# mnesbit/ImageExperiments

Measured on AMD Instinct MI355X. Metric: encode Mpixels/s at quality=3.5, higher is better.
Workload: dtype f64; 1 GPU; 4928x3264 synthetic RGB, 8 distinct frames in turn (mt19937 seed 12345+f), quality 3.5, K=32 atoms/tile-channel, 8x8 tiles; container_bytes=6650795

## Files before the change

### imageexperiments_amd/csrc/mp_pursuit.hip

```cpp
#include <hip/hip_runtime.h>
#include <stdint.h>
#include <type_traits>

#include "mp_device.h"

namespace mpc {

namespace {

constexpr int N = 64;
constexpr int kGroups = 1;
constexpr int kWavesDouble = 12;
constexpr int kWavesFloat = 12;
constexpr int kWavesMax = 16;
constexpr int kTilesLds = kBaseFilterTiles + kBlockFilterTiles;
constexpr double W_R = 0.299, W_G = 0.587, W_B = 0.114;
constexpr double U_SCALE = 0.436 / (1.0 - 0.114);
constexpr double V_SCALE = 0.615 / (1.0 - 0.299);
#ifndef MPC_SLACK
#define MPC_SLACK 0x1p-13f
#endif
constexpr float kSlack = MPC_SLACK;
constexpr float kAbs = 0x1p-100f;
constexpr float kHuge = 1.0e30f;
// ... 40 lines not shown
    unsigned lo = (unsigned)__double2loint(x), hi = (unsigned)__double2hiint(x);
    const auto a = __builtin_amdgcn_permlane16_swap(lo, lo, false, false);
    const auto b = __builtin_amdgcn_permlane16_swap(hi, hi, false, false);
    const double m = __hiloint2double((int)b[0], (int)a[0]) + __hiloint2double((int)b[1], (int)a[1]);
    lo = (unsigned)__double2loint(m); hi = (unsigned)__double2hiint(m);
    const auto c = __builtin_amdgcn_permlane32_swap(lo, lo, false, false);
    const auto d = __builtin_amdgcn_permlane32_swap(hi, hi, false, false);
    return __hiloint2double((int)d[0], (int)c[0]) + __hiloint2double((int)d[1], (int)c[1]);
}
__device__ __forceinline__ double from_prev16(double x)
{
    const unsigned lo = (unsigned)__double2loint(x), hi = (unsigned)__double2hiint(x);
    const auto a = __builtin_amdgcn_permlane16_swap(lo, lo, false, false);
    const auto b = __builtin_amdgcn_permlane16_swap(hi, hi, false, false);
    return __hiloint2double((int)b[0], (int)a[0]);
}
__device__ __forceinline__ double from_next16(double x)
{
    const unsigned lo = (unsigned)__double2loint(x), hi = (unsigned)__double2hiint(x);
    const auto a = __builtin_amdgcn_permlane16_swap(lo, lo, false, false);
    const auto b = __builtin_amdgcn_permlane16_swap(hi, hi, false, false);
    return __hiloint2double((int)b[1], (int)a[1]);
}
__device__ __forceinline__ double from_prev32(double x)
{
    const unsigned lo = (unsigned)__double2loint(x), hi = (unsigned)__double2hiint(x);
    const auto a = __builtin_amdgcn_permlane32_swap(lo, lo, false, false);
    const auto b = __builtin_amdgcn_permlane32_swap(hi, hi, false, false);
    return __hiloint2double((int)b[0], (int)a[0]);
}
__device__ __forceinline__ double from_next32(double x)
{
    const unsigned lo = (unsigned)__double2loint(x), hi = (unsigned)__double2hiint(x);
    const auto a = __builtin_amdgcn_permlane32_swap(lo, lo, false, false);
    const auto b = __builtin_amdgcn_permlane32_swap(hi, hi, false, false);
    return __hiloint2double((int)b[1], (int)a[1]);
}

__device__ __forceinline__ float from_prev16(float x) { return __uint_as_float(__builtin_amdgcn_permlane16_swap(__float_as_uint(x), __float_as_uint(x), false, false)[0]); }
__device__ __forceinline__ float from_next16(float x) { return __uint_as_float(__builtin_amdgcn_permlane16_swap(__float_as_uint(x), __float_as_uint(x), false, false)[1]); }
__device__ __forceinline__ float from_prev32(float x) { return __uint_as_float(__builtin_amdgcn_permlane32_swap(__float_as_uint(x), __float_as_uint(x), false, false)[0]); }
__device__ __forceinline__ float from_next32(float x) { return __uint_as_float(__builtin_amdgcn_permlane32_swap(__float_as_uint(x), __float_as_uint(x), false, false)[1]); }

__device__ __forceinline__ int pos_of(int h) { return h ^ (h >> 1); }

template <class T>
__device__ __forceinline__ T chain_sum(const T (&term)[16], int h)
{
    T t = 0;
#pragma unroll
    for (int i = 0; i < 16; ++i) t += term[i];
    T u = from_prev16(t);
#pragma unroll
    for (int i = 0; i < 16; ++i) u += term[i];
    t = h == 1 ? u : t;
    u = from_prev32(t);
#pragma unroll
    for (int i = 0; i < 16; ++i) u += term[i];
    t = h == 3 ? u : t;
    u = from_next16(t);
#pragma unroll
    for (int i = 0; i < 16; ++i) u += term[i];
    t = h == 2 ? u : t;
    u = from_prev16(t);
    t = h == 3 ? u : t;
    u = from_next32(t);
    return h < 2 ? u : t;
}

struct TopKeys {
    float k1 = 0.0f, k2 = 0.0f;
    __device__ __forceinline__ void see(unsigned value_bits, unsigned keep_mask, unsigned code)
    {
        const unsigned key = (value_bits & keep_mask) | code;
        k2 = __builtin_amdgcn_fmed3f(k1, k2, __uint_as_float(key));
        const unsigned k1b = __float_as_uint(k1);
        k1 = __uint_as_float(k1b > key ? k1b : key);
    }
};
__device__ __forceinline__ unsigned in_vgpr(unsigned x)
{
    unsigned v;
    asm volatile("v_mov_b32 %0, %1" : "=v"(v) : "s"(x));
    return v;
}
__device__ __forceinline__ unsigned in_sgpr(unsigned x)
{
    unsigned v;
    asm volatile("s_mov_b32 %0, %1" : "=s"(v) : "s"(x));
    return v;
}
constexpr unsigned kKeepRow = 0x7FFFFF80u;
constexpr unsigned kKeepPair = 0x7FFFFE00u;

struct Survivors {
    int q0 = 0, q1 = 0, q2 = 0, q3 = 0, count = 0;
    bool overflow = false;
    __device__ __forceinline__ void push(int code)
    {
        if (count == 0) q0 = code; else if (count == 1) q1 = code; else if (count == 2) q2 = code; else if (count == 3) q3 = code;
        else overflow = true;
        if (count < 4) ++count;
    }
    __device__ __forceinline__ int at(int i) const { return i == 0 ? q0 : (i == 1 ? q1 : (i == 2 ? q2 : q3)); }
};

struct TileChannel {
    int prev_id = 0;
    int next_off = 0;
    int off0 = 0;
    int npairs = 0;
    int fresh = -1;
    unsigned pk0 = 0, pk1 = 0;
    unsigned swept = 0;
    bool has0 = false, live = false;
    double coeff = 0.0;
    int sel_g = 0;
    int step = 0;
    int t = 0;
    __device__ __forceinline__ unsigned packed(int p) const { return ((p < 2 ? pk0 : pk1) >> (16 * (p & 1))) & 0xFFFFu; }
};

__device__ __forceinline__ void load16(double (&x)[16], const double* p)
{
    const double2* q = reinterpret_cast<const double2*>(p);
#pragma unroll
    for (int i = 0; i < 8; ++i) {
        const double2 v = q[i];
        x[2 * i] = v.x;
        x[2 * i + 1] = v.y;
    }
}

__device__ __forceinline__ void load16(float (&x)[16], const float* p)
{
    const float4* q = reinterpret_cast<const float4*>(p);
#pragma unroll
    for (int i = 0; i < 4; ++i) {
        const float4 v = q[i];
        x[4 * i] = v.x;
        x[4 * i + 1] = v.y;
        x[4 * i + 2] = v.z;
        x[4 * i + 3] = v.w;
    }
}

__device__ __forceinline__ double abs_of(double x) { return __builtin_fabs(x); }
__device__ __forceinline__ float abs_of(float x) { return __builtin_fabsf(x); }

template <class T>
__device__ __forceinline__ void keep_better(T& v, int& i, int& sel, T ov, int oi, int osel)
{
    const T a = abs_of(ov), b = abs_of(v);
    if (oi >= 0 && (a > b || (a == b && i >= 0 && oi < i))) {
        v = ov; i = oi; sel = osel;
    }
}

__device__ __forceinline__ int lane_id_fresh()
{
    int l;
    asm volatile("v_mbcnt_lo_u32_b32 %0, -1, 0\n\tv_mbcnt_hi_u32_b32 %0, -1, %0" : "=v"(l));
    return l;
}
#define FRESH_LANE                                                                    \
    const int lane = lane_id_fresh();                                                 \
    const int slot = lane & 15, h = lane >> 4;                                        \
    const int pix0 = 16 * pos_of(h);                                                  \
    (void)slot; (void)h; (void)pix0;

#ifdef MPC_STAMPS
#define STAMP(i)                                              \
// ... 38 lines not shown
            s_tiles[i] = i < kBaseFilterTiles * 256 ? src_base[i] : src_blk0[i - kBaseFilterTiles * 256];
        for (int i = threadIdx.x; i < 512; i += 64 * kWaves) {
            s_rows[i] = i < a.num_base ? a.block_rows[i] : 0;
            s_rowoff[i] = i < a.num_base ? a.block_row_off[i] : 0;
        }
        for (int i = threadIdx.x; i < 3 * kMaxDeviceK; i += 64 * kWaves)
            s_quant[i / kMaxDeviceK][i % kMaxDeviceK] = (i % kMaxDeviceK) < a.K ? a.quant[(i / kMaxDeviceK) * a.K + i % kMaxDeviceK] : 1.0;
        if (threadIdx.x == 0) {
            s_home = ch_first;
            s_on[0] = s_on[1] = s_on[2] = 0;
            s_on[ch_first] = kWaves;
        }
    }
    __syncthreads();

    const int wave = __builtin_amdgcn_readfirstlane((int)(threadIdx.x >> 6));
    int ch = ch_first;
    const T* detail = nullptr;
    const uint16_t* block_tiles = nullptr;
    const float* gram = nullptr;
    unsigned* queue = nullptr;
    long long n_tc = 0;
    auto bind_channel = [&](int c) {
        c = __builtin_amdgcn_readfirstlane(c);
        ch = c;
        detail = reinterpret_cast<const T*>(kFast ? static_cast<const void*>(c == 0 ? a.detail32[0] : (c == 1 ? a.detail32[1] : a.detail32[2]))
                                                  : static_cast<const void*>(c == 0 ? a.detail[0] : (c == 1 ? a.detail[1] : a.detail[2])));
        block_tiles = c == 0 ? a.block_tiles[0] : (c == 1 ? a.block_tiles[1] : a.block_tiles[2]);
        gram = c == 0 ? a.gram[0] : (c == 1 ? a.gram[1] : a.gram[2]);
        queue = a.queue + c;
        n_tc = c == 0 ? a.n_tc[0] : (c == 1 ? a.n_tc[1] : a.n_tc[2]);
    };
    bind_channel(ch_first);
    const long long wave_global = (long long)blockIdx.x * kWaves + wave;
    float* const my_p = a.pair_p + wave_global * (kGroups * 16 * kMaxPairs * 64);
    unsigned* const my_meta = a.pair_meta + wave_global * (kGroups * 16 * kMaxPairs * 2);
    float* const my_e = a.pair_e + wave_global * (kGroups * 16 * kMaxPairs);
    unsigned* const my_touch = s_touch + 64 * wave;
    const int K = a.K;

    const unsigned keep_row_mask = in_vgpr(kKeepRow), keep_pair_mask = in_vgpr(kKeepPair);
    unsigned n_mfma = 0, n_steps = 0;
    int unit[kGroups];
    T r[kGroups][16];
    TileChannel tc[kGroups];
#pragma unroll
    for (int g = 0; g < kGroups; ++g) {
        unit[g] = -1;
#pragma unroll
        for (int i = 0; i < 16; ++i) r[g][i] = 0;
    }
    bool queue_empty = false;

    auto tile_mfma = [&](const uint4 (&av)[4], const bf16x8 (&hi)[2], const bf16x8 (&lo)[2]) {
        f32x4 acc = {0.0f, 0.0f, 0.0f, 0.0f};
#pragma unroll
        for (int kk = 0; kk < 2; ++kk) {
            bf16x8 ah, al;
            __builtin_memcpy(&ah, &av[2 * kk + 0], 16);
            __builtin_memcpy(&al, &av[2 * kk + 1], 16);
            acc = __builtin_amdgcn_mfma_f32_16x16x32_bf16(ah, hi[kk], acc, 0, 0, 0);
            acc = __builtin_amdgcn_mfma_f32_16x16x32_bf16(ah, lo[kk], acc, 0, 0, 0);
            acc = __builtin_amdgcn_mfma_f32_16x16x32_bf16(al, hi[kk], acc, 0, 0, 0);
        }
        return acc;
    };
    auto rec_of = [&](int t) { return a.vec_in ? (long long)t : (long long)t * 3 + ch; };
    auto lds_tile = [&](uint4 (&dst)[4], int t, int lane) {
#pragma unroll
        for (int q = 0; q < 4; ++q) dst[q] = s_tiles[t * 256 + q * 64 + lane];
    };
    auto far_tile = [&](uint4 (&dst)[4], int t, int lane) {
        const uint4* tiles = reinterpret_cast<const uint4*>(block_tiles) + lane;
#pragma unroll
        for (int q = 0; q < 4; ++q) dst[q] = tiles[t * 256 + q * 64];
    };

    TopKeys tp[kGroups];
    float lbmax[kGroups];
    bool oddp[kGroups];
    float rbound[kGroups];
#pragma unroll
    for (int g = 0; g < kGroups; ++g) { lbmax[g] = -3.0e38f; oddp[g] = false; rbound[g] = 0.0f; }
    auto pair_update = [&](auto gc, auto same_p, int p, bool upd, unsigned info, float4 (&pv)[4], const float4 (&gv)[4], float E) {
        constexpr int g = decltype(gc)::value;
        FRESH_LANE
        const long long pi = (long long)(g * 16 + slot) * kMaxPairs + p;
        const int rows = (int)((info >> 9) & 127u);
        if (upd) {
            const float c32 = (float)tc[g].coeff;
            float4* pp = reinterpret_cast<float4*>(my_p + pi * 64 + 4 * h);
#pragma unroll
            for (int t = 0; t < 4; ++t) {
                pv[t].x = fmaf(-c32, gv[t].x, pv[t].x);
                pv[t].y = fmaf(-c32, gv[t].y, pv[t].y);
                pv[t].z = fmaf(-c32, gv[t].z, pv[t].z);
                pv[t].w = fmaf(-c32, gv[t].w, pv[t].w);
                pp[4 * t] = pv[t];
            }
            E = (E + 0x1p-21f * (fabsf(c32) + rbound[g])) * 1.000001f;
            if (h == 0) my_e[pi] = E;
            oddp[g] = oddp[g] || !(fabsf(c32) < kHuge);
        }
        oddp[g] = oddp[g] || !(E < kHuge);
        const bool pad2 = h == 3 && rows < 63, pad3 = h == 3 && rows < 64;
        const unsigned keepp = keep_pair_mask;
        float biggest = 0.0f;
#pragma unroll
        for (int t = 0; t < 4; ++t) {
            const float vals[4] = {pv[t].x, pv[t].y, pv[t].z, pv[t].w};
#pragma unroll
            for (int v = 0; v < 4; ++v) {
                const float m = fabsf(vals[v]);
                float ub = m + E;
                if (t == 3 && v == 2) ub = pad2 ? 0.0f : ub;
                if (t == 3 && v == 3) ub = pad3 ? 0.0f : ub;
                const unsigned code = (unsigned)((p << 4) | (t << 2) | v);
                tp[g].see(__float_as_uint(ub), keepp, decltype(same_p)::value ? in_sgpr((unsigned)__builtin_amdgcn_readfirstlane((int)code)) : code);
                biggest = __builtin_amdgcn_fmed3f(biggest, m, __builtin_inff());
            }
        }
        lbmax[g] = __builtin_amdgcn_fmed3f(lbmax[g], biggest - E, __builtin_inff());
    };
    for (;;) {
        bool any_unit = false;
        for (;;) {
        static_for<kGroups>([&](auto gc) {
            constexpr int g = decltype(gc)::value;
            if (queue_empty) return;
            const unsigned free_slots = (unsigned)(__ballot(!tc[g].live) & 0xFFFFull);
            const int n_free = __popc(free_slots);
            if (!(n_free >= kRefillAt || (unit[g] < 0 && n_free > 0))) return;
            FRESH_LANE
            int first = 0;
            if (lane == 0) first = (int)atomicAdd(queue, (unsigned)n_free);
            first = __builtin_amdgcn_readfirstlane(first);
            if ((long long)first + n_free >= n_tc) queue_empty = true;
            const long long t = (long long)first + __popc(free_slots & ((1u << slot) - 1u));
            const bool take = !tc[g].live && t < n_tc;
            if (!__ballot(take)) return;
            unit[g] = 0;
            TileChannel s;
            s.live = true;
            s.t = (int)t;
            s.next_off = a.num_base;
            const long long ts = take ? t : 0;
            T fresh_r[16];
            if (a.vec_in) {
                double in[16];
                load16(in, a.vec_in + ts * N + pix0);
#pragma unroll
                for (int i = 0; i < 16; ++i) fresh_r[i] = (T)in[i];
            } else {
                const int tiles_per_frame = a.tiles_x * a.tile_rows;
                const int frame = (int)(ts / tiles_per_frame);
                const int tile = (int)(ts - (long long)frame * tiles_per_frame);
                const int tx = tile / a.tile_rows, ty = a.tile_row_begin + (tile - tx * a.tile_rows);
                if (a.out_tile_rows > 0) s.t = (frame * a.tiles_x + tx) * a.out_tile_rows + ty;
                const uint8_t* img = a.rgb + (long long)frame * a.frame_stride;
                unsigned char px[16][3];
                const bool whole = tx * 8 + 8 <= a.width && ty * 8 + 8 <= a.height;
                if (a.rgb_aligned8 && !__ballot(!whole)) {
#pragma unroll
                    for (int rr = 0; rr < 2; ++rr) {
                        const uint2* p = reinterpret_cast<const uint2*>(img + (long long)(ty * 8 + (pix0 >> 3) + rr) * a.row_stride + 24 * tx);
                        const uint2 v0 = p[0], v1 = p[1], v2 = p[2];
                        const unsigned w[6] = {v0.x, v0.y, v1.x, v1.y, v2.x, v2.y};
#pragma unroll
                        for (int b = 0; b < 24; ++b) px[8 * rr + b / 3][b % 3] = (unsigned char)((w[b >> 2] >> (8 * (b & 3))) & 0xFFu);
                    }
                } else {
#pragma unroll
                    for (int i = 0; i < 16; ++i) {
                        const int x = tx * 8 + (i & 7), y = ty * 8 + (pix0 >> 3) + (i >> 3);
                        const int xc = x < a.width ? x : a.width - 1, yc = y < a.height ? y : a.height - 1;
                        const uint8_t* p = img + (long long)yc * a.row_stride + 3 * xc;
                        px[i][0] = p[0]; px[i][1] = p[1]; px[i][2] = p[2];
                    }
                }
#pragma unroll
                for (int i = 0; i < 16; ++i) {
                    const int x = tx * 8 + (i & 7), y = ty * 8 + (pix0 >> 3) + (i >> 3);
                    const double red = (double)px[i][0], green = (double)px[i][1], blue = (double)px[i][2];
                    const double Y = (W_R * red + W_G * green + W_B * blue);
                    const double v = ch == 0 ? Y : (ch == 1 ? (U_SCALE * (blue - Y)) : (V_SCALE * (red - Y)));
                    fresh_r[i] = (T)((x < a.width && y < a.height) ? v : 0.0);
                }
            }
            if (take) {
#pragma unroll
                for (int i = 0; i < 16; ++i) r[g][i] = fresh_r[i];
                tc[g] = s;
            }
        });
#pragma unroll
        for (int g = 0; g < kGroups; ++g) any_unit = any_unit || unit[g] >= 0;
        if (any_unit || !queue_empty) break;
        int next = ch + 1;
        while (next < 3 && (next == 1 ? a.n_tc[1] : a.n_tc[2]) == 0) ++next;
        if (next >= 3) break;
        int was_on = 0;
        FRESH_LANE
        if (lane == 0) {
            __hip_atomic_fetch_add(&s_on[next], 1, __ATOMIC_RELAXED, __HIP_MEMORY_SCOPE_WORKGROUP);
            was_on = __hip_atomic_fetch_add(&s_on[ch], -1, __ATOMIC_ACQ_REL, __HIP_MEMORY_SCOPE_WORKGROUP);
// ... 9 lines not shown
            if (lane == 0) __hip_atomic_store(&s_home, next, __ATOMIC_RELEASE, __HIP_MEMORY_SCOPE_WORKGROUP);
        }
        bind_channel(next);
        queue_empty = false;
        }
        if (!any_unit) break;
        const bool home = __builtin_amdgcn_readfirstlane(__hip_atomic_load(&s_home, __ATOMIC_ACQUIRE, __HIP_MEMORY_SCOPE_WORKGROUP)) == ch;
        static_for<kGroups>([&](auto gc) { n_steps += (unsigned)__popcll(__ballot(unit[decltype(gc)::value] >= 0 && tc[decltype(gc)::value].live) & 0xFFFFull); });
        STAMP(0)
        COUNT(12, 1)
        static_for<kGroups>([&](auto gc) { COUNT(16, __popcll(__ballot(tc[decltype(gc)::value].live && unit[decltype(gc)::value] >= 0))) });

        bf16x8 bh[kGroups][2], bl[kGroups][2];
        float Eb[kGroups], rnorm[kGroups];
        bool nz[kGroups], odd[kGroups];
        static_for<kGroups>([&](auto gc) {
            constexpr int g = decltype(gc)::value;
            double ss = 0.0;
            bool nzl = false;
#pragma unroll
            for (int i = 0; i < 16; ++i) {
                const T d = r[g][i];
                nzl = nzl || (d != 0);
                const float x = (float)d;
                ss += (double)x * (double)x;
                const unsigned short hb = bf16_of(x);
                const unsigned short lb = bf16_of(x - __uint_as_float((unsigned)hb << 16));
                bh[g][i >> 3][i & 7] = (short)hb;
                bl[g][i >> 3][i & 7] = (short)lb;
            }
            ss = reduce4_add(ss);
            nz[g] = reduce4_add(nzl ? 1u : 0u) != 0u;
            rnorm[g] = (float)__builtin_sqrt(ss) * 1.0000002f;
            Eb[g] = kSlack * rnorm[g] + kAbs;
            rbound[g] = rnorm[g];
            odd[g] = !(rnorm[g] < kHuge);
        });
        STAMP(1)

        static_for<kGroups>([&](auto gc) {
            constexpr int g = decltype(gc)::value;
            if (unit[g] < 0) return;
            const bool mine = tc[g].live && tc[g].fresh >= 0;
            unsigned long long pend = __ballot(mine) & 0xFFFFull;
            if (!pend) return;
            FRESH_LANE
            COUNT(19, __popcll(pend))
            unsigned fresh_info = 0;
            if (mine)
                fresh_info = (tc[g].fresh < 4 ? tc[g].packed(tc[g].fresh) : my_meta[2 * ((long long)(g * 16 + slot) * kMaxPairs + tc[g].fresh)]) & 0xFFFFu;
            float4 pnew[4];
#pragma unroll
            for (int t = 0; t < 4; ++t) pnew[t] = make_float4(0.0f, 0.0f, 0.0f, 0.0f);
            while (pend) {
                const int src = __builtin_ctzll(pend);
                pend &= pend - 1;
                const int blk = __builtin_amdgcn_readlane((int)(fresh_info & 511u), src);
                n_mfma += 6 * kBlockFilterTiles;
                const uint4* tiles = reinterpret_cast<const uint4*>(block_tiles) + (long long)blk * (kBlockFilterTiles * 256) + lane;
#ifndef MPC_NEWPAIR_TILES
#define MPC_NEWPAIR_TILES 2
#endif
                constexpr int kInFlight = MPC_NEWPAIR_TILES;
#pragma unroll
                for (int t2 = 0; t2 < kBlockFilterTiles; t2 += kInFlight) {
                    uint4 av[kInFlight][4];
#pragma unroll
                    for (int t = 0; t < kInFlight; ++t)
#pragma unroll
                        for (int q = 0; q < 4; ++q) av[t][q] = tiles[(t2 + t) * 256 + q * 64];
#pragma unroll
                    for (int t = 0; t < kInFlight; ++t) {
                        const f32x4 acc = tile_mfma(av[t], bh[g], bl[g]);
                        if (slot == src) pnew[t2 + t] = make_float4(acc[0], acc[1], acc[2], acc[3]);
                    }
                }
            }
            if (mine) {
                float4* dst = reinterpret_cast<float4*>(my_p + ((long long)(g * 16 + slot) * kMaxPairs + tc[g].fresh) * 64 + 4 * h);
#pragma unroll
                for (int t = 0; t < 4; ++t) dst[4 * t] = pnew[t];
                if (h == 0) my_e[(g * 16 + slot) * kMaxPairs + tc[g].fresh] = Eb[g];
                const float4 none[4] = {};
                pair_update(gc, std::false_type{}, tc[g].fresh, false, fresh_info, pnew, none, Eb[g]);
            }
        });
        STAMP(3)

        TopKeys tb[kGroups], td[kGroups];
        bool any0 = false;
#pragma unroll
        for (int g = 0; g < kGroups; ++g) any0 = any0 || (unit[g] >= 0 && __ballot(tc[g].live && tc[g].has0) != 0);
        n_mfma += 6 * kGroups * (kBaseFilterTiles + (any0 ? kBlockFilterTiles : 0));
        {
            FRESH_LANE
            uint4 ta[4];
            f32x4 acc[kGroups], prev[kGroups];
            const unsigned keep = keep_row_mask;
            auto track = [&](TopKeys (&trk)[kGroups], const f32x4 (&val)[kGroups], unsigned code0) {
                unsigned code[4];
#pragma unroll
                for (int v = 0; v < 4; ++v) code[v] = (unsigned)__builtin_amdgcn_readfirstlane((int)(code0 + v));
#pragma unroll
                for (int g = 0; g < kGroups; ++g)
#pragma unroll
                    for (int v = 0; v < 4; ++v) trk[g].see(__float_as_uint(val[g][v]), keep, code[v]);
            };
            lds_tile(ta, 0, lane);
#pragma unroll
            for (int g = 0; g < kGroups; ++g) prev[g] = tile_mfma(ta, bh[g], bl[g]);
#pragma unroll 1
            for (int t = 1; t < kBaseFilterTiles - 1; t += 2) {
                lds_tile(ta, t, lane);
#pragma unroll
                for (int g = 0; g < kGroups; ++g) acc[g] = tile_mfma(ta, bh[g], bl[g]);
                track(tb, prev, 4 * (t - 1));
                lds_tile(ta, t + 1, lane);
#pragma unroll
                for (int g = 0; g < kGroups; ++g) prev[g] = tile_mfma(ta, bh[g], bl[g]);
                track(tb, acc, 4 * t);
            }
            lds_tile(ta, kBaseFilterTiles - 1, lane);
#pragma unroll
            for (int g = 0; g < kGroups; ++g) acc[g] = tile_mfma(ta, bh[g], bl[g]);
            track(tb, prev, 4 * (kBaseFilterTiles - 2));
            track(tb, acc, 4 * (kBaseFilterTiles - 1));
            if (any0) {
#pragma unroll 1
                for (int t = 0; t < kBlockFilterTiles; ++t) {
                    if (home) lds_tile(ta, kBaseFilterTiles + t, lane);
                    else far_tile(ta, t, lane);
#pragma unroll
                    for (int g = 0; g < kGroups; ++g) acc[g] = tile_mfma(ta, bh[g], bl[g]);
                    track(td, acc, 4 * t);
                }
            }
        }
        STAMP(4)

        Survivors sv[kGroups];
        float thr_b[kGroups], Tmin[kGroups];
        bool pass2[kGroups], rescan[kGroups];
        static_for<kGroups>([&](auto gc) {
            constexpr int g = decltype(gc)::value;
            pass2[g] = false; rescan[g] = false; thr_b[g] = 0.0f; Tmin[g] = 0.0f;
            if (unit[g] < 0) return;
            FRESH_LANE
            const bool has0 = tc[g].has0, hasp = tc[g].npairs > 0;
            const float top_b = __uint_as_float(__float_as_uint(reduce4_max(tb[g].k1)) & kKeepRow);
            const float top_d = __uint_as_float(__float_as_uint(reduce4_max(td[g].k1)) & kKeepRow);
            const float lbm = reduce4_max(lbmax[g]);
            const bool bad = odd[g] || (hasp && reduce4_add(oddp[g] ? 1u : 0u) != 0u);
            float t = top_b - Eb[g];
            if (has0) t = fmaxf(t, top_d - Eb[g]);
            if (hasp) t = fmaxf(t, lbm);
            Tmin[g] = bad ? -__builtin_inff() : t;
            thr_b[g] = (Tmin[g] - Eb[g]) * (1.0f - 0x1p-15f);
            const float thr_p = Tmin[g] * (1.0f - 0x1p-13f);
            const bool live = tc[g].live && nz[g];
            const bool vague = bad || !(thr_b[g] > 0.0f);
            const bool unclear_b = vague || !(tb[g].k2 < thr_b[g]) || (has0 && !(td[g].k2 < thr_b[g]));
            const bool unclear_p = hasp && (vague || !(tp[g].k2 < thr_p));
            pass2[g] = __ballot(live && unclear_b) != 0;
            rescan[g] = live && reduce4_add(unclear_p ? 1u : 0u) != 0u;
            if (live && !pass2[g]) {
                if (!(tb[g].k1 < thr_b[g])) {
                    const unsigned code = __float_as_uint(tb[g].k1) & 127u;
// ... 167 lines not shown
                            if (on[g]) on[g] = row < (int)((my_meta[2 * ((long long)(g * 16 + slot7) * kMaxPairs + p)] >> 9) & 127u);
                        }
                        any = any || on[g];
                    });
                    if (!__ballot(more)) break;
                    if (!__ballot(any)) continue;
                    evaluate2(on, code);
                }
            }
        }
        STAMP(9)

        T xrow[kGroups][16];
#pragma unroll
        for (int g = 0; g < kGroups; ++g) {
            FRESH_LANE
            const int sg = (unit[g] >= 0 && tc[g].live && best_idx[g] >= 0) ? best_sel[g] : 0;
            load16(xrow[g], (sg < a.num_base ? base_rows + (long long)sg * N : detail + (long long)(sg - a.num_base) * N) + pix0);
        }
        bool ended[kGroups];
        static_for<kGroups>([&](auto gc) {
            constexpr int g = decltype(gc)::value;
            ended[g] = false;
            if (unit[g] < 0) return;
            FRESH_LANE
            TileChannel& s = tc[g];
            s.coeff = 0.0;
            s.fresh = -1;
            if (!s.live) return;
            s.swept += (unsigned)s.next_off;
            int count = 0;
            unsigned record = 0;
            if (best_idx[g] < 0) {
                ended[g] = true; count = s.step;
            } else {
                const int id = best_idx[g];
                const unsigned delta = s.step > 0 ? (((unsigned)(id - s.prev_id) << 1) ^ (unsigned)((id - s.prev_id) >> 31)) : (unsigned)id;
                s.prev_id = id;
                const T qstep = (T)s_quant[ch][s.step];
                const T ratio = best_val[g] / qstep;
                const int q = kFast ? (int)__builtin_roundf((float)ratio) : (int)__builtin_round((double)ratio);
                const unsigned zz = ((unsigned)q << 1) ^ (unsigned)(q >> 31);
                record = (delta & 0xFFFFu) | ((zz & 0xFFFFu) << 16);
                if (q == 0) {
                    ended[g] = true; count = s.step;
                } else {
                    s.coeff = (double)(qstep * (T)q);
                    s.sel_g = best_sel[g];
                    if (s.step + 1 == K) { ended[g] = true; count = K; }
                    else if (id < a.num_base) {
                        const int rows = s_rows[id];
                        bool repeat = id == 0 && s.has0;
                        for (int p = 0; p < s.npairs; ++p) {
                            const unsigned blk = p < 4 ? (s.packed(p) & 511u) : (my_meta[2 * ((long long)(g * 16 + slot) * kMaxPairs + p)] & 511u);
                            repeat = repeat || (int)blk == id;
                        }
                        if (!repeat) {
                            if (id == 0) { s.has0 = true; s.off0 = s.next_off; }
                            else {
                                const long long pi = (long long)(g * 16 + slot) * kMaxPairs + s.npairs;
                                const unsigned info = (unsigned)id | ((unsigned)rows << 9);
                                if (h == 0) my_meta[2 * pi] = info | ((unsigned)s.next_off << 16);
                                if (s.npairs < 2) s.pk0 |= info << (16 * s.npairs);
                                else if (s.npairs < 4) s.pk1 |= info << (16 * (s.npairs - 2));
                                s.fresh = s.npairs;
                                s.npairs += 1;
                            }
                        }
                        s.next_off += rows;
                    }
                }
            }
            if (h == 0) {
                const long long rec = rec_of(s.t);
                a.out.choices[rec * K + s.step] = record;
                if (ended[g]) {
                    a.out.counts[rec] = (uint16_t)count;
                    if (a.out.swept) a.out.swept[rec] = s.swept;
                }
            }
        });
        STAMP(10)

        float4 pv0[kGroups][4], gv0[kGroups][4];
        float E0[kGroups];
        bool on0[kGroups], upd0[kGroups];
        unsigned info0[kGroups];
#pragma unroll
        for (int g = 0; g < kGroups; ++g) {
            FRESH_LANE
            on0[g] = unit[g] >= 0 && tc[g].live && !ended[g] && tc[g].npairs > 0 && tc[g].fresh != 0;
            upd0[g] = on0[g] && tc[g].coeff != 0.0;
            info0[g] = tc[g].packed(0);
            const long long pi = (long long)(g * 16 + slot) * kMaxPairs;
            const float4* pp = reinterpret_cast<const float4*>(my_p + pi * 64 + 4 * h);
            const float4* gp = reinterpret_cast<const float4*>(gram + (upd0[g] ? (long long)tc[g].sel_g * a.gram_stride + (int)(info0[g] & 511u) * 64 : 0) + 4 * h);
#pragma unroll
            for (int t = 0; t < 4; ++t) { pv0[g][t] = pp[4 * t]; gv0[g][t] = gp[4 * t]; }
            E0[g] = my_e[pi];
        }
#pragma unroll
        for (int g = 0; g < kGroups; ++g) { tp[g] = TopKeys(); lbmax[g] = -3.0e38f; oddp[g] = false; }
        static_for<kGroups>([&](auto gc) {
            constexpr int g = decltype(gc)::value;
            if (__ballot(on0[g])) { COUNT(17, 1) COUNT(18, __popcll(__ballot(on0[g]) & 0xFFFFull)) }
            if (on0[g]) pair_update(gc, std::true_type{}, 0, upd0[g], info0[g], pv0[g], gv0[g], E0[g]);
        });
#pragma unroll 1
        for (int p = 1;; ++p) {
            bool on[kGroups];
            bool any = false;
#pragma unroll
            for (int g = 0; g < kGroups; ++g) {
                on[g] = unit[g] >= 0 && tc[g].live && !ended[g] && p < tc[g].npairs && p != tc[g].fresh;
                any = any || (unit[g] >= 0 && tc[g].live && !ended[g] && p < tc[g].npairs);
            }
            if (!__ballot(any)) break;
            unsigned info[kGroups];
            float4 pv[kGroups][4], gv[kGroups][4];
            float E[kGroups];
            bool upd[kGroups];
#pragma unroll
            for (int g = 0; g < kGroups; ++g) {
                FRESH_LANE
                const long long pi = (long long)(g * 16 + slot) * kMaxPairs + (on[g] ? p : 0);
                info[g] = p < 4 ? tc[g].packed(p) : (my_meta[2 * pi] & 0xFFFFu);
                upd[g] = on[g] && tc[g].coeff != 0.0;
                const float4* pp = reinterpret_cast<const float4*>(my_p + pi * 64 + 4 * h);
                const float4* gp = reinterpret_cast<const float4*>(gram + (upd[g] ? (long long)tc[g].sel_g * a.gram_stride + (int)(info[g] & 511u) * 64 : 0) + 4 * h);
#pragma unroll
                for (int t = 0; t < 4; ++t) { pv[g][t] = pp[4 * t]; gv[g][t] = gp[4 * t]; }
                E[g] = my_e[pi];
            }
            static_for<kGroups>([&](auto gc) {
                constexpr int g = decltype(gc)::value;
                COUNT(17, 1) COUNT(18, __popcll(__ballot(on[g]) & 0xFFFFull))
                if (on[g]) pair_update(gc, std::true_type{}, p, upd[g], info[g], pv[g], gv[g], E[g]);
            });
        }
        STAMP(2)


        static_for<kGroups>([&](auto gc) {
            constexpr int g = decltype(gc)::value;
            if (unit[g] < 0) return;
            FRESH_LANE
            TileChannel& s = tc[g];
            const bool upd = s.live && s.coeff != 0.0;
            if (upd) {
#pragma unroll
                for (int i = 0; i < 16; ++i) {
                    const T scaled = (T)s.coeff * xrow[g][i];
                    r[g][i] = r[g][i] - scaled;
                }
            }
            if (a.out.energy && __ballot(s.live && ended[g])) {
                T sq[16];
#pragma unroll
                for (int i = 0; i < 16; ++i) sq[i] = r[g][i] * r[g][i];
                const T e2 = chain_sum(sq, h);
                if (s.live && ended[g] && h == 0) a.out.energy[rec_of(s.t)] = (double)e2;
            }
            unsigned long long pend = __ballot(s.live && !ended[g] && s.fresh >= 0 && s.fresh < 4 && h == 0);
            while (pend) {
                const int src = __builtin_ctzll(pend);
                pend &= pend - 1;
                const int blk = __builtin_amdgcn_readlane((int)(s.packed(s.fresh >= 0 && s.fresh < 4 ? s.fresh : 0) & 511u), src);
                const uint16_t* tiles = block_tiles + (long long)blk * (kBlockFilterTiles * 2048) + 64 * lane;
                __builtin_amdgcn_global_load_lds(tiles, my_touch, 4, 0, 0);
                __builtin_amdgcn_global_load_lds(tiles + 4096, my_touch, 4, 0, 0);
            }
            if (ended[g]) s.live = false;
            s.step += 1;
            if (!__ballot(s.live)) unit[g] = -1;
        });
        STAMP(11)
    }
    FRESH_LANE
    if (lane == 0 && a.stats) {
        atomicAdd(a.stats + 0, (unsigned long long)n_mfma);
        atomicAdd(a.stats + 1, (unsigned long long)n_steps);
    }
#ifdef MPC_STAMPS
    if (lane == 0 && a.debug)
        for (int i = 0; i < 24; ++i) atomicAdd(a.debug + i, stamp_acc[i]);
    if (lane == 0 && a.debug && blockIdx.x < 1024) {
        atomicMin(a.debug + 24 + 2 * blockIdx.x, wg_begin);
        atomicMax(a.debug + 25 + 2 * blockIdx.x, (unsigned long long)__builtin_amdgcn_s_memrealtime());
    }
#endif
}

__global__ __launch_bounds__(256) void mp_gram_kernel(const double* __restrict__ base, const double* __restrict__ detail,
                                                      const int32_t* __restrict__ block_rows, const int32_t* __restrict__ block_row_off,
                                                      const uint8_t* __restrict__ shadow, float* __restrict__ gram, int num_base,
                                                      int n_sel, long long stride)
{
    __shared__ double sa[64][65];
    __shared__ double sb[64][65];
    const int blk = blockIdx.x, sel0 = blockIdx.y * 64;
    const int rows = block_rows[blk], off = block_row_off[blk];
    for (int i = threadIdx.x; i < 64 * 64; i += 256) {
        const int rr = i >> 6, k = i & 63;
        const int sel = sel0 + rr;
        double va = 0.0;
        if (sel < n_sel) va = sel < num_base ? base[(long long)sel * N + k] : detail[(long long)(sel - num_base) * N + k];
        sa[rr][k] = va;
        double vb = 0.0;
        if (rr < rows && !shadow[off + rr]) vb = detail[(long long)(off + rr) * N + k];
        sb[rr][k] = vb;
    }
    __syncthreads();
    const int ty = threadIdx.x >> 4, tx = threadIdx.x & 15;
    double acc[4][4];
#pragma unroll
    for (int i = 0; i < 4; ++i)
#pragma unroll
        for (int j = 0; j < 4; ++j) acc[i][j] = 0.0;
    for (int k = 0; k < N; ++k) {
        double av[4], bv[4];
#pragma unroll
        for (int i = 0; i < 4; ++i) { av[i] = sa[4 * ty + i][k]; bv[i] = sb[4 * tx + i][k]; }
#pragma unroll
        for (int i = 0; i < 4; ++i)
// ... 38 lines not shown
```

### imageexperiments_amd/csrc/mpcodec_capi.cpp

```cpp
#include "../../include/mpcodec.h"

#include <hip/hip_runtime.h>

#include <atomic>
#include <cmath>
#include <chrono>
#include <cstdarg>
#include <cstdio>
#include <cstdlib>
#include <algorithm>
#include <cstring>
#include <new>
#include <utility>
#include <stdexcept>
#include <future>
#include <memory>
#include <mutex>
#include <vector>

#include "host_bitstream.h"
#include "mpc_internal.h"
#include "host_codec.h"
#include "host_stats.h"
#include "host_dictionary.h"
// ... 316 lines not shown
    if (forced > 0) workgroups = std::min(forced, d.workgroups);
    std::lock_guard<std::mutex> hold(d.launch_lock);
    HIP_TRY(hipStreamWaitEvent(s, d.done[0], 0));
    HIP_TRY(hipMemsetAsync(d.queues, 0, 3 * sizeof(unsigned), s));
    const long long n_sel = d.num_base + d.detail_rows, stride = static_cast<long long>(d.num_base) * 64;
    mpc::PursuitArgs a{};
    a.base = d.d_base;
    a.base32 = d.d_base32;

    a.fast = c->fast ? 1 : 0;
    a.base_tiles = d.d_base_t1;
    for (int ch = 0; ch < 3; ++ch) {
        a.detail[ch] = d.d_detail + static_cast<size_t>(ch) * d.detail_rows * mpc::kTileN;
        a.detail32[ch] = d.d_detail32 + static_cast<size_t>(ch) * d.detail_rows * mpc::kTileN;
        a.block_tiles[ch] = d.d_detail_t1 + static_cast<size_t>(ch) * d.num_base * mpc::kBlockFilterTiles * mpc::kFilterTileHalves;
        a.gram[ch] = d.d_gram + static_cast<size_t>(ch) * n_sel * stride;
        a.n_tc[ch] = vec ? (ch == in.vec_channel ? n_tc : 0) : n_tc;
    }
    a.pair_p = d.pair_p;
    a.pair_meta = d.pair_meta;
    a.pair_e = d.pair_e;
    a.workgroups = workgroups;
    a.gram_stride = stride;
    a.block_rows = d.d_rows;
    a.block_row_off = d.d_rowoff;
    a.quant = d_quant;
    a.K = c->K;
    a.num_base = d.num_base;
    a.rows0 = c->dict.block_rows.empty() ? 0 : c->dict.block_rows[0];
    a.rgb = in.rgb;
    a.width = in.width;
    a.height = in.height;
    a.row_stride = in.row_stride;
    a.frame_stride = in.frame_stride;
    a.tile_row_begin = in.tile_row_begin;
    a.tile_rows = in.tile_rows;
    a.tiles_x = in.tiles_x;
    a.out_tile_rows = in.out_tile_rows;
    a.rgb_aligned8 = (reinterpret_cast<uintptr_t>(in.rgb) % 8 == 0 && in.row_stride % 8 == 0 && (in.frames <= 1 || in.frame_stride % 8 == 0)) ? 1 : 0;
    a.vec_in = in.vec_in;
    a.vec_channel = in.vec_channel;
    a.queue = d.queues;
    a.out = out;
    a.stats = d.stats;
    hipEvent_t* ev = nullptr;
    if (c->timing) {
        const size_t need = c->timing_used + 2;
        while (c->timing_events.size() < need) {
            hipEvent_t e;
            if (hipEventCreate(&e) != hipSuccess) return fail(MPC_ERR_HIP, "hipEventCreate failed");
            c->timing_events.push_back(e);
        }
        ev = c->timing_events.data() + c->timing_used;
        c->timing_used = need;
        HIP_TRY(hipEventRecord(ev[0], s));
    }
#ifdef MPC_STAMPS
    constexpr int kDebugWords = 24 + 2 * 1024;
    static unsigned long long* d_debug = nullptr;
    if (!d_debug) HIP_TRY(hipMalloc(reinterpret_cast<void**>(&d_debug), kDebugWords * sizeof(unsigned long long)));
    {
        std::vector<unsigned long long> init(kDebugWords, 0ULL);
        for (int b = 0; b < 1024; ++b) init[24 + 2 * b] = ~0ULL;
        HIP_TRY(hipStreamSynchronize(s));
        HIP_TRY(hipMemcpy(d_debug, init.data(), kDebugWords * sizeof(unsigned long long), hipMemcpyHostToDevice));
    }
    a.debug = d_debug;
#endif
    const int err = mpc::launch_pursuit(a, s);
    if (err != 0) return fail(MPC_ERR_HIP, "kernel launch failed: %s", hipGetErrorString(static_cast<hipError_t>(err)));
    if (ev) HIP_TRY(hipEventRecord(ev[1], s));
    HIP_TRY(hipEventRecord(d.done[0], s));
#ifdef MPC_STAMPS
    {
        std::vector<unsigned long long> all(kDebugWords);
        HIP_TRY(hipStreamSynchronize(s));
        HIP_TRY(hipMemcpy(all.data(), d_debug, kDebugWords * sizeof(unsigned long long), hipMemcpyDeviceToHost));
        const unsigned long long* hst = all.data();
        unsigned long long tot = 0;
        for (int i = 0; i < 12; ++i) tot += hst[i];
        std::fprintf(stderr, "[stamps wg%d] wave-steps %llu live-lanes/step %.1f pass2-groups %llu rounds %llu exhaustive %llu | cycles/wave-step:",
                     workgroups, hst[12], hst[12] ? (double)hst[16] / hst[12] / 4.0 : 0.0, hst[13], hst[14], hst[15]);
        for (int i = 0; i < 12; ++i) std::fprintf(stderr, " %d:%.0f", i, hst[12] ? (double)hst[i] / hst[12] : 0.0);
        std::fprintf(stderr, " total %.0f | pair rounds/step %.2f slots/round %.2f new pairs/step %.2f\n", hst[12] ? (double)tot / hst[12] : 0.0,
                     hst[12] ? (double)hst[17] / hst[12] : 0.0, hst[17] ? (double)hst[18] / hst[17] : 0.0, hst[12] ? (double)hst[19] / hst[12] : 0.0);
        const int grid = a.workgroups;
        unsigned long long t0 = ~0ULL, t1 = 0;
        for (int b = 0; b < grid && b < 1024; ++b) { t0 = std::min(t0, all[24 + 2 * b]); t1 = std::max(t1, all[25 + 2 * b]); }
        if (t1 > t0) {
            const double span = (double)(t1 - t0);
            double busy = 0.0;
            int slices[20] = {};
            for (int b = 0; b < grid && b < 1024; ++b) {
                busy += (double)(all[25 + 2 * b] - all[24 + 2 * b]);
                for (int k = 0; k < 20; ++k) {
                    const double mid = t0 + span * (k + 0.5) / 20.0;
                    if ((double)all[24 + 2 * b] <= mid && mid < (double)all[25 + 2 * b]) ++slices[k];
                }
            }
            std::fprintf(stderr, "[residency] span %.1f us, workgroup-time / (%d CUs x span) = %.3f | resident workgroups per 5 %% slice:", span / 100.0,
                         d.workgroups, busy / (span * d.workgroups));
            for (int k = 0; k < 20; ++k) std::fprintf(stderr, " %d", slices[k]);
            std::fprintf(stderr, "\n");
        }
    }
#endif
    return MPC_OK;
}

mpc_status run_pursuit(mpc_context* c, const mpc::FrameInput& in, const mpc::Outputs& out, const double* d_quant,
                       long long total_tc, void* stream) {
    if (!steps_path()) return run_persistent(c, in, out, d_quant, total_tc, stream);
    if (c->fast) return fail(MPC_ERR_ARGUMENT, "the float flavour runs on the persistent kernel only (unset MPC_PATH / MPC_FILTER)");
    mpc_status st = ensure_workspace(c, total_tc);
    if (st != MPC_OK) return st;
    const mpc::DictDevice dict = dict_device(c);
    hipStream_t caller = static_cast<hipStream_t>(stream);
    const long long npipes = pipes_for(c, total_tc);
    long long share = (total_tc + npipes - 1) / npipes;
    share = (share + 767) / 768 * 768;
    if (share > c->ws_cap) share = c->ws_cap;
    HIP_TRY(hipEventRecord(c->fork, caller));
    size_t used_pipes = 0;
    long long index = 0;
    for (long long begin = 0; begin < total_tc; begin += share, ++index) {
        const long long n = (total_tc - begin < share) ? total_tc - begin : share;
        auto& pipe = c->pipes[static_cast<size_t>(index % npipes)];
        if (index < npipes) {
            HIP_TRY(hipStreamWaitEvent(pipe.stream, c->fork, 0));
            ++used_pipes;
        }
        void** events = nullptr;
        if (c->timing) {
            const size_t need = c->timing_used + 2 * static_cast<size_t>(c->K);
            while (c->timing_events.size() < need) {
                hipEvent_t e;
                if (hipEventCreate(&e) != hipSuccess) return fail(MPC_ERR_HIP, "hipEventCreate failed");
                c->timing_events.push_back(e);
            }
            events = reinterpret_cast<void**>(c->timing_events.data() + c->timing_used);
            c->timing_used = need;
        }
        const int err = mpc::enqueue_pursuit(dict, pipe.ws, in, out, d_quant, c->K, begin, static_cast<int>(n),
                                             env_int("MPC_BASE_PARTS", kBaseParts), env_int("MPC_ROW_PARTS", kRowParts),
                                             env_int("MPC_SWEEP_WAVES", c->max_waves), pipe.stream, events,
                                             env_int("MPC_SIDE", 0) ? pipe.side : nullptr, pipe.fork, pipe.join);
        if (err != 0) return fail(MPC_ERR_HIP, "kernel launch failed: %s", hipGetErrorString(static_cast<hipError_t>(err)));
    }
    for (size_t i = 0; i < used_pipes; ++i) {
        HIP_TRY(hipEventRecord(c->pipes[i].done, c->pipes[i].stream));
        HIP_TRY(hipStreamWaitEvent(caller, c->pipes[i].done, 0));
    }
    return MPC_OK;
}
}

extern "C" {

const char* mpc_version(void) { return "mpcodec 0.1 (gfx950)"; }
const char* mpc_last_error(void) { return g_error; }
void mpc_set_error_text(const char* text) { std::snprintf(g_error, sizeof g_error, "%s", text ? text : ""); }

mpc_status mpc_context_create(int K, int block_size, double bpp, int device, mpc_context** out) {
    return guarded([&]() -> mpc_status {
    if (!out) return fail(MPC_ERR_ARGUMENT, "out is null");
    *out = nullptr;
    if (K < 1 || K > MPC_MAX_K) return fail(MPC_ERR_ARGUMENT, "K=%d out of range 1..%d", K, MPC_MAX_K);
// ... 1740 lines not shown
```

Before: 5284 Mpixels/s.

## Compact pair updates across tile-channel slots with DPP prefix scan and segmented merge

Replaces the per-pair loop, in which each of the 16 slots handled its own pair p in lockstep, with a work-compacted scheme. A DPP prefix sum over per-slot pair counts lets every lane process one (owner, pair) item from a flattened list. Per-item top-2 keys, lower bounds and odd flags are then combined with a segmented DPP reduction and gathered back into the owning slot through ds_bpermute. The aim is to stop lanes idling when slots have uneven pair counts, at the cost of extra cross-lane permutes, owner lookups and merge logic on every round.

```diff
diff --git a/imageexperiments_amd/csrc/mp_pursuit.hip b/imageexperiments_amd/csrc/mp_pursuit.hip
--- a/imageexperiments_amd/csrc/mp_pursuit.hip
+++ b/imageexperiments_amd/csrc/mp_pursuit.hip
@@ -146,12 +146,6 @@
 {
     unsigned v;
     asm volatile("v_mov_b32 %0, %1" : "=v"(v) : "s"(x));
-    return v;
-}
-__device__ __forceinline__ unsigned in_sgpr(unsigned x)
-{
-    unsigned v;
-    asm volatile("s_mov_b32 %0, %1" : "=s"(v) : "s"(x));
     return v;
 }
 constexpr unsigned kKeepRow = 0x7FFFFF80u;
@@ -356,13 +350,11 @@
     float rbound[kGroups];
 #pragma unroll
     for (int g = 0; g < kGroups; ++g) { lbmax[g] = -3.0e38f; oddp[g] = false; rbound[g] = 0.0f; }
-    auto pair_update = [&](auto gc, auto same_p, int p, bool upd, unsigned info, float4 (&pv)[4], const float4 (&gv)[4], float E) {
-        constexpr int g = decltype(gc)::value;
+    auto pair_update = [&](TopKeys& trk, float& lbm, bool& odd, long long pi, unsigned pc, bool upd, float c32, float rb,
+                           unsigned info, float4 (&pv)[4], const float4 (&gv)[4], float E) {
         FRESH_LANE
-        const long long pi = (long long)(g * 16 + slot) * kMaxPairs + p;
         const int rows = (int)((info >> 9) & 127u);
         if (upd) {
-            const float c32 = (float)tc[g].coeff;
             float4* pp = reinterpret_cast<float4*>(my_p + pi * 64 + 4 * h);
 #pragma unroll
             for (int t = 0; t < 4; ++t) {
@@ -372,11 +364,11 @@
                 pv[t].w = fmaf(-c32, gv[t].w, pv[t].w);
                 pp[4 * t] = pv[t];
             }
-            E = (E + 0x1p-21f * (fabsf(c32) + rbound[g])) * 1.000001f;
+            E = (E + 0x1p-21f * (fabsf(c32) + rb)) * 1.000001f;
             if (h == 0) my_e[pi] = E;
-            oddp[g] = oddp[g] || !(fabsf(c32) < kHuge);
-        }
-        oddp[g] = oddp[g] || !(E < kHuge);
+            odd = odd || !(fabsf(c32) < kHuge);
+        }
+        odd = odd || !(E < kHuge);
         const bool pad2 = h == 3 && rows < 63, pad3 = h == 3 && rows < 64;
         const unsigned keepp = keep_pair_mask;
         float biggest = 0.0f;
@@ -389,12 +381,15 @@
                 float ub = m + E;
                 if (t == 3 && v == 2) ub = pad2 ? 0.0f : ub;
                 if (t == 3 && v == 3) ub = pad3 ? 0.0f : ub;
-                const unsigned code = (unsigned)((p << 4) | (t << 2) | v);
-                tp[g].see(__float_as_uint(ub), keepp, decltype(same_p)::value ? in_sgpr((unsigned)__builtin_amdgcn_readfirstlane((int)code)) : code);
+                trk.see(__float_as_uint(ub), keepp, pc | (unsigned)((t << 2) | v));
                 biggest = __builtin_amdgcn_fmed3f(biggest, m, __builtin_inff());
             }
         }
-        lbmax[g] = __builtin_amdgcn_fmed3f(lbmax[g], biggest - E, __builtin_inff());
+        lbm = __builtin_amdgcn_fmed3f(lbm, biggest - E, __builtin_inff());
+    };
+    auto merge_keys = [](unsigned& k1, unsigned& k2, unsigned o1, unsigned o2) {
+        k2 = max(min(k1, o1), max(k2, o2));
+        k1 = max(k1, o1);
     };
     for (;;) {
         bool any_unit = false;
@@ -570,7 +565,8 @@
                 for (int t = 0; t < 4; ++t) dst[4 * t] = pnew[t];
                 if (h == 0) my_e[(g * 16 + slot) * kMaxPairs + tc[g].fresh] = Eb[g];
                 const float4 none[4] = {};
-                pair_update(gc, std::false_type{}, tc[g].fresh, false, fresh_info, pnew, none, Eb[g]);
+                pair_update(tp[g], lbmax[g], oddp[g], (long long)(g * 16 + slot) * kMaxPairs + tc[g].fresh, (unsigned)tc[g].fresh << 4,
+                            false, 0.0f, 0.0f, fresh_info, pnew, none, Eb[g]);
             }
         });
         STAMP(3)
@@ -904,64 +900,86 @@
         });
         STAMP(10)
 
-        float4 pv0[kGroups][4], gv0[kGroups][4];
-        float E0[kGroups];
-        bool on0[kGroups], upd0[kGroups];
-        unsigned info0[kGroups];
-#pragma unroll
-        for (int g = 0; g < kGroups; ++g) {
-            FRESH_LANE
-            on0[g] = unit[g] >= 0 && tc[g].live && !ended[g] && tc[g].npairs > 0 && tc[g].fresh != 0;
-            upd0[g] = on0[g] && tc[g].coeff != 0.0;
-            info0[g] = tc[g].packed(0);
-            const long long pi = (long long)(g * 16 + slot) * kMaxPairs;
-            const float4* pp = reinterpret_cast<const float4*>(my_p + pi * 64 + 4 * h);
-            const float4* gp = reinterpret_cast<const float4*>(gram + (upd0[g] ? (long long)tc[g].sel_g * a.gram_stride + (int)(info0[g] & 511u) * 64 : 0) + 4 * h);
-#pragma unroll
-            for (int t = 0; t < 4; ++t) { pv0[g][t] = pp[4 * t]; gv0[g][t] = gp[4 * t]; }
-            E0[g] = my_e[pi];
-        }
 #pragma unroll
         for (int g = 0; g < kGroups; ++g) { tp[g] = TopKeys(); lbmax[g] = -3.0e38f; oddp[g] = false; }
         static_for<kGroups>([&](auto gc) {
             constexpr int g = decltype(gc)::value;
-            if (__ballot(on0[g])) { COUNT(17, 1) COUNT(18, __popcll(__ballot(on0[g]) & 0xFFFFull)) }
-            if (on0[g]) pair_update(gc, std::true_type{}, 0, upd0[g], info0[g], pv0[g], gv0[g], E0[g]);
+            if (unit[g] < 0) return;
+            const int n_own = (tc[g].live && !ended[g]) ? tc[g].npairs - (tc[g].fresh >= 0 ? 1 : 0) : 0;
+            int incl = n_own;
+            incl += __builtin_amdgcn_update_dpp(0, incl, 0x111, 0xF, 0xF, true);
+            incl += __builtin_amdgcn_update_dpp(0, incl, 0x112, 0xF, 0xF, true);
+            incl += __builtin_amdgcn_update_dpp(0, incl, 0x114, 0xF, 0xF, true);
+            incl += __builtin_amdgcn_update_dpp(0, incl, 0x118, 0xF, 0xF, true);
+            const int total = __builtin_amdgcn_readlane(incl, 15);
+            if (total == 0) return;
+            const int excl = incl - n_own;
+            const unsigned owners = (unsigned)(__ballot(n_own > 0) & 0xFFFFull);
+            int span = 0;
+            for (unsigned m = owners; m; m &= m - 1) span = max(span, __builtin_amdgcn_readlane(n_own, __builtin_ctz(m)));
+#pragma unroll 1
+            for (int f0 = 0; f0 < total; f0 += 16) {
+                FRESH_LANE
+                COUNT(17, 1) COUNT(18, min(16, total - f0))
+                const int f = f0 + slot;
+                int owner = 0, first = 0;
+                for (unsigned m = owners; m; m &= m - 1) {
+                    const int s = __builtin_ctz(m), e = __builtin_amdgcn_readlane(excl, s);
+                    if (f >= e) { owner = s; first = e; }
+                }
+                const bool on = f < total;
+                const int p = on ? f - first : 0;
+                const int src = (owner + 16 * h) << 2;
+                const float c32 = __int_as_float(__builtin_amdgcn_ds_bpermute(src, __float_as_int((float)tc[g].coeff)));
+                const float rb = __int_as_float(__builtin_amdgcn_ds_bpermute(src, __float_as_int(rbound[g])));
+                const int sel = __builtin_amdgcn_ds_bpermute(src, tc[g].coeff != 0.0 ? tc[g].sel_g : -1);
+                const unsigned w0 = (unsigned)__builtin_amdgcn_ds_bpermute(src, (int)tc[g].pk0);
+                const unsigned w1 = (unsigned)__builtin_amdgcn_ds_bpermute(src, (int)tc[g].pk1);
+                const long long pi = (long long)(g * 16 + owner) * kMaxPairs + p;
+                const unsigned info = p < 4 ? ((p < 2 ? w0 : w1) >> (16 * (p & 1))) & 0xFFFFu : (my_meta[2 * pi] & 0xFFFFu);
+                const bool upd = on && sel >= 0;
+                float4 pv[4], gv[4];
+                const float4* pp = reinterpret_cast<const float4*>(my_p + pi * 64 + 4 * h);
+                const float4* gp = reinterpret_cast<const float4*>(gram + (upd ? (long long)sel * a.gram_stride + (int)(info & 511u) * 64 : 0) + 4 * h);
+#pragma unroll
+                for (int t = 0; t < 4; ++t) { pv[t] = pp[4 * t]; gv[t] = gp[4 * t]; }
+                TopKeys it;
+                float lb = -3.0e38f;
+                bool odd_it = false;
+                pair_update(it, lb, odd_it, pi, 0u, upd, c32, rb, info, pv, gv, my_e[pi]);
+                unsigned k1 = __float_as_uint(it.k1) | ((unsigned)p << 4), k2 = __float_as_uint(it.k2) | ((unsigned)p << 4);
+                unsigned od = odd_it ? 1u : 0u;
+                static_for<4>([&](auto ic) {
+                    constexpr int d = 1 << decltype(ic)::value;
+                    if (d >= span) return;
+                    const bool same = __builtin_amdgcn_update_dpp(-1, owner, 0x110 + d, 0xF, 0xF, false) == owner;
+                    const unsigned o1 = (unsigned)__builtin_amdgcn_update_dpp(0, (int)k1, 0x110 + d, 0xF, 0xF, true);
+                    const unsigned o2 = (unsigned)__builtin_amdgcn_update_dpp(0, (int)k2, 0x110 + d, 0xF, 0xF, true);
+                    const unsigned oo = (unsigned)__builtin_amdgcn_update_dpp(0, (int)od, 0x110 + d, 0xF, 0xF, true);
+                    const float ol = __int_as_float(__builtin_amdgcn_update_dpp(0, __float_as_int(lb), 0x110 + d, 0xF, 0xF, true));
+                    if (same) {
+                        merge_keys(k1, k2, o1, o2);
+                        lb = __builtin_amdgcn_fmed3f(lb, ol, __builtin_inff());
+                        od |= oo;
+                    }
+                });
+                const int lo = max(excl, f0), hi = min(incl, f0 + 16);
+                const int last = ((lo < hi ? hi - 1 - f0 : 0) + 16 * h) << 2;
+                const unsigned m1 = (unsigned)__builtin_amdgcn_ds_bpermute(last, (int)k1);
+                const unsigned m2 = (unsigned)__builtin_amdgcn_ds_bpermute(last, (int)k2);
+                const unsigned mo = (unsigned)__builtin_amdgcn_ds_bpermute(last, (int)od);
+                const float ml = __int_as_float(__builtin_amdgcn_ds_bpermute(last, __float_as_int(lb)));
+                if (lo < hi) {
+                    unsigned t1 = __float_as_uint(tp[g].k1), t2 = __float_as_uint(tp[g].k2);
+                    merge_keys(t1, t2, m1, m2);
+                    tp[g].k1 = __uint_as_float(t1);
+                    tp[g].k2 = __uint_as_float(t2);
+                    lbmax[g] = __builtin_amdgcn_fmed3f(lbmax[g], ml, __builtin_inff());
+                    oddp[g] = oddp[g] || mo != 0u;
+                }
+            }
         });
-#pragma unroll 1
-        for (int p = 1;; ++p) {
-            bool on[kGroups];
-            bool any = false;
-#pragma unroll
-            for (int g = 0; g < kGroups; ++g) {
-                on[g] = unit[g] >= 0 && tc[g].live && !ended[g] && p < tc[g].npairs && p != tc[g].fresh;
-                any = any || (unit[g] >= 0 && tc[g].live && !ended[g] && p < tc[g].npairs);
-            }
-            if (!__ballot(any)) break;
-            unsigned info[kGroups];
-            float4 pv[kGroups][4], gv[kGroups][4];
-            float E[kGroups];
-            bool upd[kGroups];
-#pragma unroll
-            for (int g = 0; g < kGroups; ++g) {
-                FRESH_LANE
-                const long long pi = (long long)(g * 16 + slot) * kMaxPairs + (on[g] ? p : 0);
-                info[g] = p < 4 ? tc[g].packed(p) : (my_meta[2 * pi] & 0xFFFFu);
-                upd[g] = on[g] && tc[g].coeff != 0.0;
-                const float4* pp = reinterpret_cast<const float4*>(my_p + pi * 64 + 4 * h);
-                const float4* gp = reinterpret_cast<const float4*>(gram + (upd[g] ? (long long)tc[g].sel_g * a.gram_stride + (int)(info[g] & 511u) * 64 : 0) + 4 * h);
-#pragma unroll
-                for (int t = 0; t < 4; ++t) { pv[g][t] = pp[4 * t]; gv[g][t] = gp[4 * t]; }
-                E[g] = my_e[pi];
-            }
-            static_for<kGroups>([&](auto gc) {
-                constexpr int g = decltype(gc)::value;
-                COUNT(17, 1) COUNT(18, __popcll(__ballot(on[g]) & 0xFFFFull))
-                if (on[g]) pair_update(gc, std::true_type{}, p, upd[g], info[g], pv[g], gv[g], E[g]);
-            });
-        }
         STAMP(2)
-
 
         static_for<kGroups>([&](auto gc) {
             constexpr int g = decltype(gc)::value;
diff --git a/imageexperiments_amd/csrc/mpcodec_capi.cpp b/imageexperiments_amd/csrc/mpcodec_capi.cpp
--- a/imageexperiments_amd/csrc/mpcodec_capi.cpp
+++ b/imageexperiments_amd/csrc/mpcodec_capi.cpp
@@ -422,7 +422,7 @@
         std::fprintf(stderr, "[stamps wg%d] wave-steps %llu live-lanes/step %.1f pass2-groups %llu rounds %llu exhaustive %llu | cycles/wave-step:",
                      workgroups, hst[12], hst[12] ? (double)hst[16] / hst[12] / 4.0 : 0.0, hst[13], hst[14], hst[15]);
         for (int i = 0; i < 12; ++i) std::fprintf(stderr, " %d:%.0f", i, hst[12] ? (double)hst[i] / hst[12] : 0.0);
-        std::fprintf(stderr, " total %.0f | pair rounds/step %.2f slots/round %.2f new pairs/step %.2f\n", hst[12] ? (double)tot / hst[12] : 0.0,
+        std::fprintf(stderr, " total %.0f | pair rounds/step %.2f items/round %.2f new pairs/step %.2f\n", hst[12] ? (double)tot / hst[12] : 0.0,
                      hst[12] ? (double)hst[17] / hst[12] : 0.0, hst[17] ? (double)hst[18] / hst[17] : 0.0, hst[12] ? (double)hst[19] / hst[12] : 0.0);
         const int grid = a.workgroups;
         unsigned long long t0 = ~0ULL, t1 = 0;
```

New measurement: 5310 Mpixels/s, median of 6. No clear change (+0.5%).
